# zyang1580/PDA

Measured on AMD Instinct MI355X. Metric: users/sec full-catalogue top-K@50 (eval), higher is better.
Workload: dtype f32; 1 GPU; C3: synthetic 1000000 users x 200000 items, d=128, PDA condition ((elu+1)*pop^0.22) head, masked top-K@50; ranks_seen=1

## Files before the change

### include/pda_hip_experimental.h

```cpp
#ifndef PDA_HIP_EXPERIMENTAL_H
#define PDA_HIP_EXPERIMENTAL_H

#include "pda_hip.h"

#ifdef __cplusplus
extern "C" {
#endif

int pda_score_topk_huge_splits(int n_users_blk, int n_items_local, int d);

int pda_topk_kth_value(const uint64_t* keys, int n_splits, int n_users_blk, int K, int pos, float* out, void* stream);
int pda_topk_remap_items(uint64_t* keys, size_t n_keys, const int32_t* gid, int n_gid, void* stream);
int pda_topk_seed_bounds(const uint64_t* keys, int n_splits, int n_users_blk, int K, int m, float* bounds, void* stream);
int pda_topk_seed_counts(const uint64_t* keys, int n_splits, int n_users_blk, int K, const float* bounds, int n_thr, int32_t* counts,
                         void* stream);
int pda_topk_seed_pick(const float* bounds, const int32_t* counts, int n_thr, int n_users_blk, int K, float* seed, void* stream);
int pda_topk_seed_refine(const uint64_t* keys, int n_splits, int n_users_blk, int K, float* lo, float* hi, float* mid, int32_t* counts,
                         int mode, void* stream);
int pda_score_topk4_phase_f32(const float* U, const float* I_shard, const void* prep, const float* pop_shard, const int32_t* users,
                              int n_users_blk, int item_offset, int n_items_local, int d, const int64_t* hist_indptr,
                              const int32_t* hist_indices, int hist_row_mode, int K, int head, int early_stop, int n_splits,
                              int phase, int warm_tiles, const float* seed, uint64_t* out_keys, void* workspace, void* stream);
int pda_score_topk4_phase_bf16(const uint16_t* U, const uint16_t* I_shard, const void* prep, const float* pop_shard,
                               const int32_t* users, int n_users_blk, int item_offset, int n_items_local, int d,
                               const int64_t* hist_indptr, const int32_t* hist_indices, int hist_row_mode, int K, int head,
                               int early_stop, int n_splits, int phase, int warm_tiles, const float* seed, uint64_t* out_keys,
                               void* workspace, void* stream);

size_t pda_triplet_plan_bytes(int B);
size_t pda_triplet_plan_large_workspace_bytes(int B);
int pda_triplet_plan_large(const int32_t* users, const int32_t* pos, const int32_t* neg, int B, void* plan, void* workspace, void* stream);
size_t pda_bpr_step_plan_scratch_bytes(int B, int d);
int pda_triplet_plan(const int32_t* users, const int32_t* pos, const int32_t* neg, int B, int n_batches, void* plans, void* stream);
int pda_bpr_step_plan_f32(float* U, float* I, const int32_t* users, const int32_t* pos, const int32_t* neg, const float* pos_pop,
                          const float* neg_pop, int B, int d, float regs, float reg_div, float lr, const void* plan, float* scratch,
                          int exact, float* loss_acc, void* stream);
int pda_bpr_step_plan_bf16(uint16_t* U_bf16, uint16_t* I_bf16, float* U_master, float* I_master, const int32_t* users,
                           const int32_t* pos, const int32_t* neg, const float* pos_pop, const float* neg_pop, int B, int d,
                           float regs, float reg_div, float lr, const void* plan, float* scratch, float* loss_acc, void* stream);

int pda_sort_triplets_by_pos(int32_t* users, int32_t* pos, int32_t* neg, float* pos_pop, float* neg_pop, int B,
                             void* stream);
// ... 59 lines not shown
```

### pda_amd/_lib.py

```python
from __future__ import annotations

import ctypes as C
import os

_HERE = os.path.dirname(os.path.abspath(__file__))
LIB_PATH = os.environ.get("PDA_HIP_LIB") or os.path.join(_HERE, "csrc", "libpda_hip.so")

ABI_VERSION = 2
HEAD_RAW, HEAD_POP = 0, 1
HIST_BY_BLOCK_ROW, HIST_BY_USER_ID = 0, 1
UPD_NONE, UPD_SGD_FUSED, UPD_DENSE_GRAD = 0, 1, 2
UPD_ANY_ORDER = 0x100
UPD_USERS_DISTINCT = 0x200
ADAM_REPLAY_FAST = 0x10
MAX_K = 64
TOPK_CAP = 60

_vp, _i, _f, _u64, _sz = C.c_void_p, C.c_int, C.c_float, C.c_uint64, C.c_size_t

class ScorePlan(C.Structure):
    _fields_ = [("path", _i), ("sweep_mode", _i), ("n_splits", _i), ("early_stop", _i), ("order", _i), ("prep_with_pop", _i),
                ("workspace_bytes", _sz), ("keys_rows", _sz)]


# ... 37 lines not shown
    "pda_score_topk4_bf16": (_i, [_vp, _vp, _vp, _vp, _vp, _i, _i, _i, _i, _vp, _vp, _i, _i, _i, _i, _i, _vp, _vp, _vp]),
    "pda_peak_mfma_flops_per_launch": (C.c_double, [_i]),
    "pda_peak_mfma_bf16": (_i, [_vp, _i, _vp]),
    "pda_peak_mfma_bf16_const": (_i, [_vp, _i, _vp]),
    "pda_peak_mfma_lds_flops_per_launch": (C.c_double, [_i]),
    "pda_peak_mfma_lds_bf16": (_i, [_vp, _sz, _vp, _i, _vp]),
    "pda_peak_copy": (_i, [_vp, _vp, _sz, _vp]),
    "pda_topk_kth_value": (_i, [_vp, _i, _i, _i, _i, _vp, _vp]),
    "pda_topk_remap_items": (_i, [_vp, _sz, _vp, _i, _vp]),
    "pda_topk_seed_refine": (_i, [_vp, _i, _i, _i, _vp, _vp, _vp, _vp, _i, _vp]),
    "pda_topk_seed_bounds": (_i, [_vp, _i, _i, _i, _i, _vp, _vp]),
    "pda_topk_seed_counts": (_i, [_vp, _i, _i, _i, _vp, _i, _vp, _vp]),
    "pda_topk_seed_pick": (_i, [_vp, _vp, _i, _i, _i, _vp, _vp]),
    "pda_score_topk4_phase_f32": (_i, [_vp, _vp, _vp, _vp, _vp, _i, _i, _i, _i, _vp, _vp, _i, _i, _i, _i, _i, _i, _i, _vp, _vp, _vp, _vp]),
    "pda_score_topk4_phase_bf16": (_i, [_vp, _vp, _vp, _vp, _vp, _i, _i, _i, _i, _vp, _vp, _i, _i, _i, _i, _i, _i, _i, _vp, _vp, _vp, _vp]),
    "pda_score_topk_plan": (_i, [_i, _i, _i, _i, _i, _i, _i, _i, _vp]),
    "pda_score_topk_huge_splits": (_i, [_i, _i, _i]),
    "pda_score_topk7_workspace_bytes": (_sz, [_i, _i, _i]),
    "pda_score_topk7_f32": (_i, [_vp, _vp, _vp, _vp, _i, _i, _i, _i, _vp, _vp, _i, _i, _i, _vp, _vp, _vp]),
    "pda_score_topk7_bf16": (_i, [_vp, _vp, _vp, _vp, _i, _i, _i, _i, _vp, _vp, _i, _i, _i, _vp, _vp, _vp]),
    "pda_topk_merge": (_i, [_vp, _i, _i, _i, _vp, _vp, _vp, _vp, _vp, _vp, _i, _vp]),
    "pda_bpr_step_f32": (_i, [_vp, _vp, _vp, _vp, _vp, _vp, _vp, _i, _i, _f, _f, _f, _i, _vp, _vp, _vp, _vp, _vp, _vp, _vp]),
    "pda_triplet_plan_bytes": (_sz, [_i]),
    "pda_bpr_step_plan_scratch_bytes": (_sz, [_i, _i]),
    "pda_triplet_plan": (_i, [_vp, _vp, _vp, _i, _i, _vp, _vp]),
    "pda_triplet_plan_large_workspace_bytes": (_sz, [_i]),
    "pda_triplet_plan_large": (_i, [_vp, _vp, _vp, _i, _vp, _vp, _vp]),
    "pda_bpr_step_plan_f32": (_i, [_vp, _vp, _vp, _vp, _vp, _vp, _vp, _i, _i, _f, _f, _f, _vp, _vp, _i, _vp, _vp]),
    "pda_bpr_step_plan_bf16": (_i, [_vp, _vp, _vp, _vp, _vp, _vp, _vp, _vp, _vp, _i, _i, _f, _f, _f, _vp, _vp, _vp, _vp]),
    "pda_sgd_apply_f32": (_i, [_vp, _vp, _vp, _vp, _vp, _vp, _vp, _vp, _i, _i, _f, _vp]),
# ... 101 lines not shown
```

### pda_amd/csrc/pda_score_topk.hip

```cpp
#include "pda_topk_common.h"
#include "pda_hip_temp_pop.h"
#include "pda_hip_pc.h"
#include <cstdlib>

namespace {

using namespace pda_topk;

template <int D, int HEAD, int ABL = 0, bool BF = false>
__global__ void __launch_bounds__(kThreads, (D <= 128 ? 2 : 1)) score_topk_kernel(ScoreArgs a) {
    extern __shared__ __attribute__((aligned(16))) unsigned char smem[];
    float* Bt = reinterpret_cast<float*>(smem);
    uint64_t* lists = reinterpret_cast<uint64_t*>(smem + 32 * D * sizeof(float));

    constexpr int CPR = D / 4;
    constexpr int NLD = (32 * CPR) / kThreads;
    static_assert(NLD >= 1, "embed dim too small for the 256-thread staging pattern");
    constexpr int NC = D / 8;
    static_assert(NC % 2 == 0, "embed dim must be a multiple of 16");

    const int tid = threadIdx.x, lane = tid & 63, wave = tid >> 6;
    const int j = lane & 31, h = lane >> 5;
    const int split = blockIdx.x % a.n_splits, utile = blockIdx.x / a.n_splits;
    const int K = a.K;
// ... 417 lines not shown
                if (a.out_val) a.out_val[(size_t)u * K + lane] = k ? pda_key_val(k) : -INFINITY;
            }
        }
        if (nreal < K && a.out_idx && a.hist_indptr && lane == 0) {
            const int64_t hr = a.hist_row_mode == PDA_HIST_BY_USER_ID ? (int64_t)a.users[u] : (int64_t)u;
            int fill = nreal, prev = -1;
            for (int64_t p = a.hist_indptr[hr]; p < a.hist_indptr[hr + 1] && fill < K; ++p) {
                const int it = a.hist_indices[p];
                if (it != prev) a.out_idx[(size_t)u * K + fill++] = it;
                prev = it;
            }
        }
    }
}

}

int pda_topk::launch_score_bias(const ScoreArgs& a, int d, hipStream_t s) {
    switch (d) {
        case 64: return launch_score<64, PDA_HEAD_BIAS>(a, s);
        case 128: return launch_score<128, PDA_HEAD_BIAS>(a, s);
        case 256: return launch_score<256, PDA_HEAD_BIAS>(a, s);
        default: return PDA_ERR_UNSUPPORTED;
    }
}

int pda_topk::launch_score_pc(const ScoreArgs& a, int d, bool by_g, hipStream_t s) {
    switch (d) {
        case 64: return by_g ? launch_score<64, kHeadPcG>(a, s) : launch_score<64, PDA_HEAD_PC>(a, s);
        case 128: return by_g ? launch_score<128, kHeadPcG>(a, s) : launch_score<128, PDA_HEAD_PC>(a, s);
// ... 63 lines not shown
    if (head != PDA_HEAD_RAW && head != PDA_HEAD_POP) return PDA_ERR_ARG;
    if (head == PDA_HEAD_POP && !pop_shard) return PDA_ERR_ARG;
    if (hist_indptr && !hist_indices) return PDA_ERR_ARG;
    if (n_splits <= 0) n_splits = pda_score_topk_auto_splits(n_users_blk, n_items_local);
    ScoreArgs a{U, I_shard, pop_shard, users, hist_indptr, hist_indices, out_keys,
                n_users_blk, item_offset, n_items_local, hist_row_mode, K, n_splits, nullptr};
    return pda_topk::launch_score_v1(a, d, head, reinterpret_cast<hipStream_t>(stream));
}

extern "C" int pda_topk_merge(const uint64_t* in_keys, int R, int n_users_blk, int K, uint64_t* out_keys,
                              int32_t* out_idx, float* out_val, const int32_t* users, const int64_t* hist_indptr,
                              const int32_t* hist_indices, int hist_row_mode, void* stream) {
    if (!in_keys || R < 1 || n_users_blk <= 0 || K < 1 || K > PDA_MAX_K) return PDA_ERR_ARG;
    if (!out_keys && !out_idx) return PDA_ERR_ARG;
    if (hist_indptr && (!hist_indices || (hist_row_mode == PDA_HIST_BY_USER_ID && !users))) return PDA_ERR_ARG;
    const size_t smem = 4 * (((size_t)R * K + PDA_MAX_K) * sizeof(uint64_t) + (((size_t)R * 4 + 7) & ~(size_t)7));
    if (smem > 160 * 1024) return PDA_ERR_UNSUPPORTED;
    static int attr_set = 0;
    if (!attr_set) {
        if (hipFuncSetAttribute(reinterpret_cast<const void*>(&topk_merge_kernel),
                                hipFuncAttributeMaxDynamicSharedMemorySize, 160 * 1024) != hipSuccess)
            return PDA_ERR_LAUNCH;
        attr_set = 1;
    }
    MergeArgs a{in_keys, out_keys, out_idx, out_val, users, hist_indptr, hist_indices, hist_row_mode, R, n_users_blk, K};
    const int blocks = min((n_users_blk + 3) / 4, 256 * 8);
    hipLaunchKernelGGL(topk_merge_kernel, dim3((unsigned)blocks), dim3(256), smem, reinterpret_cast<hipStream_t>(stream), a);
    PDA_CHECK_LAUNCH();
    return PDA_OK;
}
// ... 1 lines not shown
```

### pda_amd/csrc/pda_score_topk_v4.hip

```cpp
#include "pda_v4_shared.h"
#include <cstdlib>
#include <type_traits>

using namespace pda_topk;

namespace {

constexpr int kCap4 = 57;
constexpr int kRing4 = 128;
constexpr int kWarmTiles = 4;
constexpr int kMainWaves = 8;
#ifndef PDA_W4_ABL
#define PDA_W4_ABL 0
#endif
#ifndef PDA_V4_ABL
#define PDA_V4_ABL 0
#endif
#ifdef PDA_V4_PROF
__device__ unsigned long long pda_prof4[24];
#define PROF_T0(v) const long long v = __builtin_readcyclecounter()
#define PROF_T1(v, slot) prof[slot] += (unsigned long long)(__builtin_readcyclecounter() - v)
#define PROF_INC(slot, x) prof[slot] += (unsigned long long)(x)
#define PROF_FLUSH(first, last) do { if (lane == 0) for (int pq = (first); pq <= (last); ++pq) atomicAdd(&pda_prof4[pq], prof[pq]); } while (0)
#else
// ... 30 lines not shown
    int warm_tiles;
    int warm_sorted;
    uint64_t* handover;
    const unsigned char* rows5;
    const float* meta5;
    const unsigned char* ufrag;
    const float* unorm;
    int prep_hdr_pop;
    int warm_final;
    int warm_shared;
    float* seed_out;
    const int* n_users_dev;
    int lists_empty;
    const float* tailA;
    const float* tailB;
};


template <int D, bool BF>
__global__ void __launch_bounds__(256) prep4_kernel(const void* __restrict__ I, const float* __restrict__ pop, const int* __restrict__ order,
                                                    int n, int n_pad, unsigned char* __restrict__ rows, int* __restrict__ pos_of,
                                                    int* __restrict__ hdr, unsigned char* __restrict__ rows5, int* __restrict__ meta5, u32x4* __restrict__ pinfo,
                                                    int f16img) {
    constexpr int TPR = D / 8, RB = row_bytes(D);
    const int pos = blockIdx.x * (256 / TPR) + threadIdx.x / TPR, e = threadIdx.x % TPR;
    if (pos >= n_pad) return;
    unsigned char* rp = rows + (size_t)pos * RB;
    float ss = 0.f, popv = 1.0f, rs = 0.f;
    int src = -1;
    if (pos < n) {
// ... 336 lines not shown
    for (int q = tid; q < kUserTile * 2 * kWarmTiles; q += kThreads) hmask[q] = 0u;
    __syncthreads();
    if (g.hmask_ws != nullptr) {
        const uint32_t* src = g.hmask_ws + (size_t)blockIdx.x * kUserTile * 2 * kWarmTiles;
        for (int q = tid; q < kUserTile * 2 * kWarmTiles; q += kThreads) hmask[q] = src[q];
    } else if (g.hist_indptr != nullptr && !(PDA_W4_ABL & 1)) {
        warm_hist_walk(g, hmask, utile, split, nwarm, wave, lane);
    }
    f32x4 areg[NC];
#pragma unroll
    for (int c = 0; c < NC; ++c) {
        f32x4 v = {0.f, 0.f, 0.f, 0.f};
        if (row_ok) v = pda_load4<BF>(g.U, (size_t)uid * D + 4 * h + 8 * c);
        areg[c] = v;
    }
    if (g.pred_ws != nullptr) {
        float ss = 0.f;
#pragma unroll
        for (int c = 0; c < NC; ++c) ss += areg[c][0] * areg[c][0] + areg[c][1] * areg[c][1] + areg[c][2] * areg[c][2] + areg[c][3] * areg[c][3];
        ss += __shfl_xor(ss, 32, 64);
        if (h == 0) nul[wave * 32 + j] = sqrtf(ss) * 1.0009765625f * 1.0001f;
    }
    const float* brow = Bt + j * D;
    const int bswz = swz<D>(j);
    uint64_t* my_lists = lists + (size_t)(wave * 32) * CAP;
    constexpr int NHT = 2 * kWarmTiles;
    static_assert(NHT == 8, "eight named half-tile registers below");
    typedef uint32_t u32x16 __attribute__((ext_vector_type(16)));
    u32x16 o0 = 0u, o1 = 0u, o2 = 0u, o3 = 0u, o4 = 0u, o5 = 0u, o6 = 0u, o7 = 0u;
    int i0 = 0, i1 = 0, i2 = 0, i3 = 0, i4 = 0, i5 = 0, i6 = 0, i7 = 0;
// ... 39 lines not shown
#pragma unroll
        for (int r = 0; r < 16; ++r) {
            const int row = (r & 3) + 8 * (r >> 2) + 4 * h;
            float sc = accx[r];
            if constexpr (HEAD == PDA_HEAD_POP) sc = (sc > 0.0f ? sc + 1.0f : __expf(sc)) * pv;
            bool p = okw && (sc >= -INFINITY);
            if (any_hb) {
                const uint32_t hbr = (uint32_t)__shfl((int)hb_mine, row, 64);
                if ((hbr >> j) & 1u) p = false;
            }
            o0[r] = p ? pda_ordf(sc + 0.0f) : 0u;
        }
    }
    const u32x16 ordv[NHT] = {o0, o1, o2, o3, o4, o5, o6, o7};
    const int itemv[NHT] = {i0, i1, i2, i3, i4, i5, i6, i7};
    const int cap_t = (g.warm_sorted || g.handover != nullptr) ? CAP : K;
    auto emit_row = [&](const int r, const uint32_t t, const int c_t) __attribute__((always_inline)) {
        const int row = (r & 3) + 8 * (r >> 2) + 4 * h;
        const int lrow = wave * 32 + row;
        if (j == 0) predt[lrow] = c_t >= K ? pda_unordf(t) : -INFINITY;
        if (__any(c_t > cap_t)) {
#pragma unroll
            for (int k = 0; k < NHT; ++k) {
                const bool p = ordv[k][r] >= t;
                const uint64_t key = ((uint64_t)ordv[k][r] << 32) | (uint64_t)(0xFFFFFFFFu - (uint32_t)itemv[k]);
                append_keys<CAP>(p, lrow, pda_unordf(ordv[k][r]), key, lists, cntl, taul, wave * 32, 32, K, lane);
            }
        } else {
            int run = 0;
#pragma unroll
            for (int k = 0; k < NHT; ++k) {
// ... 85 lines not shown
    }
    pda_wave_sync();
    if (tid == 0) atomicAdd(reinterpret_cast<unsigned long long*>(g.stats + 2), (unsigned long long)(2 * nwarm));
    for (int rr = 0; rr < 32; ++rr) {
        uint64_t* buf = my_lists + rr * CAP;
        if (((PDA_W4_ABL & 4) == 0) && (g.warm_sorted || g.warm_final || (g.handover == nullptr && __builtin_amdgcn_readfirstlane(cntl[wave * 32 + rr]) > K)))
            compact_list<CAP>(buf, &cntl[wave * 32 + rr], &taul[wave * 32 + rr], K, lane);
        const int c = cntl[wave * 32 + rr];
        const int rb = utile * kUserTile + wave * 32 + rr;
        if (g.seed_out != nullptr) {
            uint32_t mn = lane < c ? (uint32_t)(buf[lane] >> 32) : 0xFFFFFFFFu;
#pragma unroll
            for (int o = 32; o >= 1; o >>= 1) mn = min(mn, (uint32_t)__shfl_xor((int)mn, o, 64));
            if (lane == 0 && rb < g.n_users_blk) g.seed_out[rb] = c >= K ? pda_unordf(mn) : -INFINITY;
        }
        if (g.handover != nullptr) {
            if (rb < g.n_users_blk && lane < CAP) g.handover[((size_t)split * g.n_users_blk + rb) * CAP + lane] = lane < c ? buf[lane] : 0ull;
            if (g.warm_final && rb < g.n_users_blk && lane < K) g.out_keys[((size_t)split * g.n_users_blk + rb) * K + lane] = lane < c ? buf[lane] : 0ull;
        } else if (rb < g.n_users_blk && lane < K) {
            const uint64_t k = lane < c ? buf[lane] : 0ull;
            g.out_keys[((size_t)split * g.n_users_blk + rb) * K + lane] = k;
        }
    }
    if (g.pred_ws != nullptr && lane < 32) {
        const int rb = utile * kUserTile + wave * 32 + lane;
        if (rb < g.n_users_blk) {
            g.pred_ws[2 * (size_t)rb] = predt[wave * 32 + lane];
            g.pred_ws[2 * (size_t)rb + 1] = nul[wave * 32 + lane];
        }
    }
}


#include "pda_v4_block_asm.h"
#ifndef PDA_V4_ASM
#define PDA_V4_ASM 1
// ... 1085 lines not shown
    {
        if constexpr (HEAD == PDA_HEAD_POP) {
            if (geometry == 4 && g.sufA == nullptr && g.prep_hdr_pop != 0) return launch_sweep5<D, BF, true, D == 256 ? 128 : 256>(g, stream);
        }
        if constexpr (D <= 128) {
            if (geometry == 3) return launch_sweep4<D, HEAD, BF, 3>(g, stream);
        }
        return launch_sweep4<D, HEAD, BF, 0>(g, stream);
    }
    return PDA_OK;
}

int user_tile4(int d) { return d == 64 ? Geo4<64>::UT : d == 128 ? Geo4<128>::UT : Geo4<256>::UT; }
static bool lists_in_hbm4(int) { return true; }
struct Ws4 {
    size_t lists, bloom, hmask, regroup, handover, ufrag, unorm, seed, total;
};
static Ws4 ws4_layout(int n_users_blk, int d, int n_splits) {
    auto al = [](size_t x) { return (x + 255) & ~(size_t)255; };
    Ws4 w{};
    w.lists = al(pda_score_topk_workspace_bytes(n_users_blk));
    size_t b = w.lists;
    if (lists_in_hbm4(d)) {
        const size_t ut = 1024;
        b += ((size_t)n_users_blk + ut - 1) / ut * (size_t)n_splits * ut * kCap4 * 8 + 256;
    }
    w.bloom = al(b);
    w.hmask = al(w.bloom + (size_t)n_users_blk * 128);
    w.regroup = al(w.hmask + ((size_t)n_users_blk + kUserTile - 1) / kUserTile * (size_t)n_splits * kUserTile * 2 * kWarmTiles * 4);
    w.handover = al(w.regroup + (1024 + 4 * (size_t)n_users_blk) * 4);
    w.total = w.handover + (size_t)n_splits * (size_t)n_users_blk * kCap4 * 8;
    w.ufrag = al(w.total);
    w.unorm = w.ufrag;
    {
        const size_t n_pad = ((size_t)n_users_blk + kUT5 - 1) / kUT5 * kUT5;
        w.unorm = w.ufrag + al(n_pad * 2 * (size_t)d);
        w.total = w.unorm + al(n_pad * 4);
    }
    w.seed = w.total;
    w.total = w.seed + al((size_t)n_users_blk * 4);
    return w;
}
extern "C" size_t pda_score_topk4_workspace_bytes(int n_users_blk, int n_items_local, int d, int n_splits) {
    if (n_users_blk <= 0 || n_items_local <= 0 || (d != 64 && d != 128 && d != 256)) return 0;
    if (n_splits <= 0) n_splits = pda_score_topk4_auto_splits(n_users_blk, n_items_local, d);
    return ws4_layout(n_users_blk, d, n_splits).total;
}

int run_score4(const void* U, const void* I_shard, bool bf16, const void* prep, const float* pop_shard, const int32_t* users,
               int n_users_blk, int item_offset, int n_items_local, int d, const int64_t* hist_indptr, const int32_t* hist_indices,
               int hist_row_mode, int K, int head, int early_stop, int n_splits, uint64_t* out_keys, void* workspace, hipStream_t s,
               int phase = 3, const float* seed = nullptr, int warm_tiles = 0, const int* n_users_dev = nullptr) {
    if (!U || !I_shard || !prep || !users || !out_keys || !workspace) return PDA_ERR_ARG;
    if (n_users_blk <= 0 || n_items_local <= 0 || item_offset < 0) return PDA_ERR_ARG;
    if (K < 1 || K > PDA_MAX_K) return PDA_ERR_ARG;
// ... 33 lines not shown
            early_stop ? sA : nullptr, early_stop ? sB : nullptr, reinterpret_cast<const int*>(pb + L.pos_of),
            reinterpret_cast<unsigned*>(workspace), reinterpret_cast<uint64_t*>(wsb + W.lists), nullptr, nullptr, nullptr, nullptr, nullptr, reinterpret_cast<const int*>(pb + L.hdr), seed, n_users_blk, item_offset, n_items_local, hist_row_mode, K, n_splits, L.n_tiles, warm_tiles,
#ifdef PDA_V4_WARM_SORTED
            1, nullptr, pb + L.rows5, reinterpret_cast<const float*>(pb + L.meta5), nullptr, nullptr, 0};
#else
            (phase == 1 || (L.n_tiles + n_splits - 1) / n_splits <= warm_tiles) ? 1 : 0, nullptr,
            pb + L.rows5, reinterpret_cast<const float*>(pb + L.meta5), nullptr, nullptr, 0};
#endif
    if (phase == 3 && !g.warm_sorted && PDA_V4_HANDOVER_WS) g.handover = reinterpret_cast<uint64_t*>(wsb + W.handover);
    g.ufrag = wsb + W.ufrag;
    g.unorm = reinterpret_cast<const float*>(wsb + W.unorm);
    g.prep_hdr_pop = (head == PDA_HEAD_POP && pop_shard != nullptr) ? 1 : 0;
    g.warm_final = (geometry >= 4 && phase == 3 && g.handover != nullptr && g.prep_hdr_pop && !early_stop) ? 1 : 0;
    g.lists_empty = from_empty ? 1 : 0;
    g.n_users_dev = n_users_dev;
    if (g.prep_hdr_pop) {
        g.tailA = reinterpret_cast<const float*>(pb + L.sufA);
        g.tailB = reinterpret_cast<const float*>(pb + L.sufB);
    }
    if (phase == 3 && n_splits > 1 && seed == nullptr && !warm_per_split && L.n_tiles > n_splits * warm_tiles) {
        g.warm_shared = 1;
        g.seed_out = reinterpret_cast<float*>(wsb + W.seed);
    }
    if (hist_indptr && (phase & 2)) {
        uint32_t* bloom = reinterpret_cast<uint32_t*>(wsb + W.bloom);
        hipLaunchKernelGGL(hist_bloom4_kernel, dim3((unsigned)((n_users_blk + 31) / 32)), dim3(256), 0, s, users, hist_indptr, hist_indices,
                           hist_row_mode, n_users_blk, bloom, reinterpret_cast<const int*>(pb + L.hdr), head == PDA_HEAD_POP ? 1 : 0);
        PDA_CHECK_LAUNCH();
        g.bloom = bloom;
    }
// ... 249 lines not shown

extern "C" int pda_score_topk4_f32(const float* U, const float* I_shard, const void* prep, const float* pop_shard, const int32_t* users,
                                   int n_users_blk, int item_offset, int n_items_local, int d, const int64_t* hist_indptr,
                                   const int32_t* hist_indices, int hist_row_mode, int K, int head, int early_stop, int n_splits,
                                   uint64_t* out_keys, void* workspace, void* stream) {
    return run_score4(U, I_shard, false, prep, pop_shard, users, n_users_blk, item_offset, n_items_local, d, hist_indptr, hist_indices,
                      hist_row_mode, K, head, early_stop, n_splits, out_keys, workspace, reinterpret_cast<hipStream_t>(stream));
}
extern "C" int pda_score_topk4_bf16(const uint16_t* U, const uint16_t* I_shard, const void* prep, const float* pop_shard, const int32_t* users,
                                    int n_users_blk, int item_offset, int n_items_local, int d, const int64_t* hist_indptr,
                                    const int32_t* hist_indices, int hist_row_mode, int K, int head, int early_stop, int n_splits,
                                    uint64_t* out_keys, void* workspace, void* stream) {
    return run_score4(U, I_shard, true, prep, pop_shard, users, n_users_blk, item_offset, n_items_local, d, hist_indptr, hist_indices,
                      hist_row_mode, K, head, early_stop, n_splits, out_keys, workspace, reinterpret_cast<hipStream_t>(stream));
}
```

### pda_amd/csrc/pda_v5_sweep.h

```cpp
#pragma once
#ifdef PDA_V6_LOOP_HEADER
#include PDA_V6_LOOP_HEADER
#else
#include "pda_v6_loop_asm.h"
#endif
#include "pda_v6_free_asm.h"

#ifdef PDA_V5_LOG
__device__ unsigned pda_v5_log[1 << 18];
#define V5LOG(kind, a, b) do { if (lane == 0) { const unsigned i_ = atomicAdd(&pda_v5_log[0], 1u); if (i_ < (1u << 16) - 1u) { \
    pda_v5_log[4 * i_ + 4] = ((unsigned)blockIdx.x << 8) | (unsigned)wave; pda_v5_log[4 * i_ + 5] = (kind); pda_v5_log[4 * i_ + 6] = (a); pda_v5_log[4 * i_ + 7] = (b); } } } while (0)
#else
#define V5LOG(kind, a, b) do {} while (0)
#endif
constexpr int kRing5 = 192;



template <int D, bool BF, bool S16, int UPW>
__global__ void __launch_bounds__(256, 1) sweep5_kernel(Args4 g) {
    [[maybe_unused]] constexpr int HB = half_bytes5(D);
    static_assert(slot_bytes5(D) == Loop6<D, 8>::kSlotBytes, "one LDS image for all loops");
    static_assert(S16, "the loop on v_mfma_f32_32x32x16_bf16 (round 4's first form: 9.16 against 8.07 ms, profiles/README.md) left with round 5; the parameter keeps the kernel's name");
    static_assert((D <= 128 && UPW == 256) || (D == 256 && UPW == 128), "users per wave: 256, or (d = 256) 128 -- 8 blocks x 8 k-steps = 256 AGPRs, one 512-user workgroup per CU");
// ... 17 lines not shown
    const int K = g.K;
    const int nt = split_tiles(g.n_tiles, split, g.n_splits);
    const int wt = warm_tiles_of(g, split);
    const bool starts_empty = g.lists_empty || (g.warm_shared && split > 0);
    const bool warm_final = g.warm_final && !starts_empty;
    const int n_it = max(0, nt - wt);
    const unsigned hend = 2u * (unsigned)n_it;
    if (tid < 72) sync[tid] = (tid < 8 || tid >= 40 || warm_final || starts_empty) ? 0u : 0xFFFFFFFFu;
    if (tid == 0 && blockIdx.x == 0) g.stats[4] = (4u << 28) | (4u << 8) | (1u << 13) | ((BF ? 1u : 0u) << 14) | (unsigned)(D >> 6);
    if (starts_empty) {
        for (int rr = tid; rr < UT; rr += 256) {
            cntl[rr] = 0;
            taul[rr] = utile * UT + rr < g.n_users_blk ? -INFINITY : INFINITY;
        }
        __builtin_amdgcn_fence(__ATOMIC_RELEASE, "workgroup");
    } else if (warm_final) {
        for (int rr = tid; rr < UT; rr += 256) {
            const int rb = utile * UT + rr;
            int c = 0;
            float tau = INFINITY;
            if (rb < g.n_users_blk) {
                const uint64_t kl = lists[(size_t)rr * CAPL + (K - 1)];
                c = K;
                tau = pda_unordf((uint32_t)(kl >> 32));
                if (kl == 0ull) {
                    tau = -INFINITY;
                    for (c = 0; c < K - 1 && lists[(size_t)rr * CAPL + c] != 0ull; ++c) {}
                }
            }
            cntl[rr] = c;
// ... 45 lines not shown
            const int rb = utile * UT + row0 + UBW * u + j;
            eu = fmaxf(eu, rb < g.n_users_blk ? g.unorm[rb] : 0.f);
            seedv[u] = (g.seed != nullptr && rb < g.n_users_blk) ? g.seed[rb] : -INFINITY;
        }
#pragma unroll
        for (int o = 32; o >= 1; o >>= 1) eu = fmaxf(eu, __shfl_xor(eu, o, 64));
        const float numax = eu;
        eu = __int_as_float(__builtin_amdgcn_readfirstlane(__float_as_int(eu * (kEps5 * 1.001f))));
        const unsigned ring_lds = (unsigned)(size_t)(__attribute__((address_space(3))) unsigned char*)tiles;
        const unsigned flags_lds = (unsigned)(size_t)(__attribute__((address_space(3))) unsigned char*)reinterpret_cast<unsigned char*>(sync);
        uint64_t* my_ring = crings + wave * kRing5;
        unsigned ring_n = 0;
        const unsigned t0 = (unsigned)(split + wt * g.n_splits);
        const size_t img = (size_t)g.rows5, meta = (size_t)g.meta5;
        const bool hist_on = g.hist_indptr != nullptr;

        auto thr_of = [&](int u) __attribute__((always_inline)) -> float {
            const float tq = fmaxf(taul[row0 + UBW * u + j], seedv[u]);
            float tf = (tq == INFINITY || tq == -INFINITY) ? tq : tq - fabsf(tq) * 1.52587890625e-5f - 1e-30f;
            return fminf(fmaxf(tf, -1.0e30f), 1.0e30f);
        };
        auto rescore_ring = [&]() __attribute__((always_inline)) {
            const int q = lane % LPC, ci = lane / LPC;
            for (unsigned base = 0; base < ring_n; base += CPP) {
                const bool have = base + (unsigned)ci < ring_n;
                const uint64_t e = have ? my_ring[base + ci] : 0ull;
                const int row = (int)(e >> 32);
                const unsigned pos = (unsigned)e;
                bool valid = have && pos < (unsigned)g.n_items_local;
                const unsigned char* tail = g.rows + (size_t)(valid ? pos : 0u) * RB4 + 2 * D + 32;
// ... 77 lines not shown
                const float o0 = LPC == 8 ? o_other : __int_as_float(__builtin_amdgcn_mov_dpp(__float_as_int(o), 0xB1, 0xF, 0xF, true));
                float sc = o0 + o;
                sc = (sc > 0.0f ? sc + 1.0f : __expf(sc)) * pv;
                const float tt = (valid && q == LPC - 1) ? sc : -INFINITY;
                const int item = g.item_offset + loc;
                bool p = valid && q == LPC - 1 && (tt >= fmaxf(c_tau, c_sd));
                if (hist_on && p) {
                    long long lo = hb, hi2 = he;
                    while (lo < hi2) {
                        const long long mid = (lo + hi2) >> 1;
                        if (g.hist_indices[mid] < item) lo = mid + 1; else hi2 = mid;
                    }
                    if (lo < he && g.hist_indices[lo] == item) p = false;
                }
                const uint64_t key = pda_pack_key(tt, (uint32_t)item);
                if (p) atomicOr(&touched[(row0 + row) >> 5], 1u << ((row0 + row) & 31));
                append_keys<CAPL, true>(p, row0 + row, tt, key, lists, cntl, taul, row0, UPW, K, lane, s_uns);
            }
            n_cand += ring_n;
            ring_n = 0;
        };
        auto extract = [&](unsigned ft) __attribute__((always_inline)) {
            const unsigned T = t0 + (ft >> 1) * (unsigned)g.n_splits;
            const unsigned pos0 = T * 64u + (ft & 1u) * 32u;
            const float2 mt = *reinterpret_cast<const float2*>(g.meta5 + 4 * (size_t)(2u * T + (ft & 1u)));
            const float ct = __builtin_fmaf(eu, mt.y, mt.x);
            const unsigned char* tb = tiles + (ft & (kNSlot5 - 1)) * SS + j * (2 * D);
            auto item_of = [&](int r) __attribute__((always_inline)) -> unsigned {
                return 16u * (r >> 2) + 4u * hh + (r & 3);
            };
            constexpr int NR = 8;
// ... 187 lines not shown
}

template <int D, bool BF, bool S16, int UPW>
int launch_sweep5(const Args4& g, hipStream_t stream) {
    constexpr int UT = 4 * UPW;
    constexpr size_t lds = (size_t)kNSlot5 * slot_bytes5(D) + (size_t)UT * 8 + 4 * kRing5 * 8 + 80 * 4 + 64;
    static_assert(UPW == 256 || D == 256 || 2 * lds <= 160 * 1024, "two workgroups per CU");
    static_assert(lds <= 160 * 1024, "LDS per workgroup");
    static int attr_set = 0;
    if (!attr_set) {
        if (hipFuncSetAttribute(reinterpret_cast<const void*>(&sweep5_kernel<D, BF, S16, UPW>), hipFuncAttributeMaxDynamicSharedMemorySize, (int)lds) != hipSuccess)
            return PDA_ERR_LAUNCH;
        attr_set = 1;
    }
    const int utiles = (g.n_users_blk + UT - 1) / UT, n_pad = utiles * UT;
    hipLaunchKernelGGL((uprep5_kernel<D, BF, S16, UPW>), dim3((unsigned)(((size_t)n_pad * (D / 8) + 255) / 256)), dim3(256), 0, stream, g.U, g.users, g.n_users_blk, n_pad,
                       const_cast<unsigned char*>(g.ufrag), const_cast<float*>(g.unorm));
    PDA_CHECK_LAUNCH();
    hipLaunchKernelGGL((sweep5_kernel<D, BF, S16, UPW>), dim3((unsigned)(utiles * g.n_splits)), dim3(256), lds, stream, g);
    PDA_CHECK_LAUNCH();
    return PDA_OK;
}
```

### pda_amd/ops.py

```python
from __future__ import annotations

import math
import os
from typing import Optional, Tuple

import ctypes as C

import torch

from . import _lib
from ._lib import (HEAD_POP, HEAD_RAW, HIST_BY_BLOCK_ROW, HIST_BY_USER_ID, UPD_ANY_ORDER, UPD_DENSE_GRAD, UPD_NONE, UPD_USERS_DISTINCT,
                   UPD_SGD_FUSED, check, ptr, stream_ptr)

ADAM_BETA1, ADAM_BETA2, ADAM_EPS = 0.9, 0.999, 1e-8


def _need(t: Optional[torch.Tensor], dtype, name: str, optional=False):
    if t is None:
        if optional:
            return None
        raise ValueError(f"{name} is required")
    if not t.is_cuda:
        raise ValueError(f"{name} must live in HBM (cuda tensor); pda_amd has no CPU path")
    if t.dtype != dtype:
# ... 504 lines not shown
        check(fn(ptr(U), ptr(I_shard), ptr(prep), ptr(pop_shard), ptr(users), nu, item_offset, nloc, d,
                 ptr(hist.indptr) if hist else None, ptr(hist.indices) if hist else None, hist.mode if hist else 0,
                 K, head, es, n_splits, ptr(out), ptr(ws), stream_ptr()), "pda_score_topk4")
        if os.environ.get("PDA_CHECK_SWEEP_ERRORS"):
            err = int(ws[0:4].view(torch.int32)[0])
            if err != 0:
                raise RuntimeError("pda_score_topk4: the sweep reported protocol error %d" % err)
        if stats is not None:
            stats["tiles_scored"] = ws[8:16].view(torch.int64)
            stats["pairs_rescored"] = ws[4:8].view(torch.int32)
            stats["tiles_dense"] = ((nloc + 31) // 32) * ((nu + 127) // 128)
            stats["kernel_id"] = ws[16:20].view(torch.int32)
            stats["huge_entries"] = ws[20:24].view(torch.int32)
            stats["huge_free_halftiles"] = ws[28:32].view(torch.int32)
            stats["error"] = ws[0:4].view(torch.int32)
        return out
    if impl == "v2" and prune:
        prep, order = item_prep_ordered(I_shard, pop_shard if head == HEAD_POP else None)
        hist_ord = hist_reordered(hist, prep, order, item_offset, nloc, d) if hist else None
        ws = torch.empty(lib.pda_score_topk_workspace_bytes(nu), dtype=torch.uint8, device=U.device)
        fn = lib.pda_score_topk_ordered_bf16 if bf else lib.pda_score_topk_ordered_f32
        check(fn(ptr(U), ptr(I_shard), ptr(prep), ptr(pop_shard), ptr(users), nu, item_offset,
                                             nloc, d, ptr(hist.indptr) if hist else None,
                                             ptr(hist.indices) if hist else None, ptr(hist_ord), hist.mode if hist else 0,
                                             K, head, 0 if prune == "order" else 1, n_splits, ptr(out), ptr(ws), stream_ptr()),
              "pda_score_topk_ordered")
        if stats is not None:
            stats["tiles_scored"] = ws[8:16].view(torch.int64)
            stats["pairs_rescored"] = ws[4:8].view(torch.int32)
            stats["tiles_dense"] = ((nloc + 31) // 32) * ((nu + 127) // 128)
# ... 72 lines not shown
        stats["error"] = ws[0:4].view(torch.int32)
        stats["fallback_rows"] = ws[24:28].view(torch.int32)
        stats["workspace"] = ws
    return out


GEOMETRY_NAMES = {0: "lds", 3: "many", 4: "huge", 7: "funnel"}


def kernel_identity(word) -> dict:
    w = int(word) & 0xFFFFFFFF
    if w == 0:
        return {"generation": 0}
    return {"generation": w >> 28, "geometry": GEOMETRY_NAMES.get((w >> 8) & 15, "?") if (w >> 28) == 4 else None,
            ("early_stop" if (w >> 28) == 4 else "visiting_order"): bool((w >> 12) & 1), "head": (w >> 13) & 1, "bf16": bool((w >> 14) & 1), "d": (w & 15) * 64}


def topk_merge(keys: torch.Tensor, users=None, hist: Optional[HistoryCSR] = None, want="idx_val"):
    lib = _lib.load()
    keys = _need(keys, torch.int64, "keys")
    R, nu, K = keys.shape
    dev = keys.device
    out_keys = out_idx = out_val = None
    if want == "keys":
        out_keys = torch.empty((nu, K), dtype=torch.int64, device=dev)
    else:
        out_idx = torch.empty((nu, K), dtype=torch.int32, device=dev)
        out_val = torch.empty((nu, K), dtype=torch.float32, device=dev)
    if users is not None:
        users = _need(users, torch.int32, "users")
# ... 847 lines not shown
```

Baseline: 32.05 million users/s.

## Fuse user-image prep into warm phase, drop handover copy, add R=1 unpack

The warm-phase kernel now writes the bf16 user fragment image and user norms itself, so the sweep no longer launches a separate uprep kernel. The final warm phase stores only the per-split K-th value plus the K keys instead of a full CAP-wide handover list. The sweep then reloads a row's list lazily, only the first time that row gains a candidate. A vectorised single-split unpack kernel replaces the shared-memory merge when R==1. Together these aim to cut extra launches and HBM traffic, in exchange for more complex sweep logic (ballot-driven lazy reloads with extra syncs) and new correctness risk in list reconstruction.

Result: faster. 32.42 million users/s, median of 6 (+1.2%).

```diff
diff --git a/include/pda_hip_experimental.h b/include/pda_hip_experimental.h
--- a/include/pda_hip_experimental.h
+++ b/include/pda_hip_experimental.h
@@ -26,6 +26,9 @@
                                const int64_t* hist_indptr, const int32_t* hist_indices, int hist_row_mode, int K, int head,
                                int early_stop, int n_splits, int phase, int warm_tiles, const float* seed, uint64_t* out_keys,
                                void* workspace, void* stream);
+int pda_score_topk4_phase_image_offsets(int n_users_blk, int n_items_local, int d, int n_splits, size_t* offs);
+int pda_score_topk4_phase_user_image(const void* U, int bf16, const int32_t* users, int n_users_blk, int d, void* ufrag, float* unorm,
+                                     void* stream);
 
 size_t pda_triplet_plan_bytes(int B);
 size_t pda_triplet_plan_large_workspace_bytes(int B);
diff --git a/pda_amd/_lib.py b/pda_amd/_lib.py
--- a/pda_amd/_lib.py
+++ b/pda_amd/_lib.py
@@ -75,6 +75,8 @@
     "pda_topk_seed_pick": (_i, [_vp, _vp, _i, _i, _i, _vp, _vp]),
     "pda_score_topk4_phase_f32": (_i, [_vp, _vp, _vp, _vp, _vp, _i, _i, _i, _i, _vp, _vp, _i, _i, _i, _i, _i, _i, _i, _vp, _vp, _vp, _vp]),
     "pda_score_topk4_phase_bf16": (_i, [_vp, _vp, _vp, _vp, _vp, _i, _i, _i, _i, _vp, _vp, _i, _i, _i, _i, _i, _i, _i, _vp, _vp, _vp, _vp]),
+    "pda_score_topk4_phase_image_offsets": (_i, [_i, _i, _i, _i, _vp]),
+    "pda_score_topk4_phase_user_image": (_i, [_vp, _i, _vp, _i, _i, _vp, _vp, _vp]),
     "pda_score_topk_plan": (_i, [_i, _i, _i, _i, _i, _i, _i, _i, _vp]),
     "pda_score_topk_huge_splits": (_i, [_i, _i, _i]),
     "pda_score_topk7_workspace_bytes": (_sz, [_i, _i, _i]),
diff --git a/pda_amd/csrc/pda_score_topk.hip b/pda_amd/csrc/pda_score_topk.hip
--- a/pda_amd/csrc/pda_score_topk.hip
+++ b/pda_amd/csrc/pda_score_topk.hip
@@ -455,6 +455,74 @@
     }
 }
 
+constexpr int kUnpackKeys = 4;
+
+__device__ __forceinline__ void unpack1_fill_row(const MergeArgs& a, size_t u) {
+    const int K = a.K;
+    const uint64_t* row = a.in_keys + u * K;
+    int nreal = 0;
+    for (int p = 0; p < K; ++p) nreal += row[p] != 0ull ? 1 : 0;
+    int32_t* orow = a.out_idx + u * K;
+    for (int p = 0; p < K; ++p)
+        if (row[p] == 0ull) orow[p] = -1;
+    const int64_t hr = a.hist_row_mode == PDA_HIST_BY_USER_ID ? (int64_t)a.users[u] : (int64_t)u;
+    int fill = nreal, prev = -1;
+    for (int64_t p = a.hist_indptr[hr]; p < a.hist_indptr[hr + 1] && fill < K; ++p) {
+        const int it = a.hist_indices[p];
+        if (it != prev) orow[fill++] = it;
+        prev = it;
+    }
+}
+
+__global__ void __launch_bounds__(256) topk_unpack1_kernel(MergeArgs a, size_t total) {
+    typedef uint64_t u64x2 __attribute__((ext_vector_type(2)));
+    typedef int32_t i32x4 __attribute__((ext_vector_type(4)));
+    const size_t g = (size_t)blockIdx.x * 256 + threadIdx.x;
+    const size_t i0 = g * kUnpackKeys;
+    if (i0 >= total) return;
+    const bool fill_on = a.out_idx != nullptr && a.hist_indptr != nullptr;
+    if (i0 + kUnpackKeys <= total) {
+        const u64x2 k01 = *reinterpret_cast<const u64x2*>(a.in_keys + i0), k23 = *reinterpret_cast<const u64x2*>(a.in_keys + i0 + 2);
+        const uint64_t k[kUnpackKeys] = {k01[0], k01[1], k23[0], k23[1]};
+        if (a.out_keys) {
+            *reinterpret_cast<u64x2*>(a.out_keys + i0) = k01;
+            *reinterpret_cast<u64x2*>(a.out_keys + i0 + 2) = k23;
+        }
+        if (a.out_idx == nullptr) return;
+        i32x4 id;
+        f32x4 v;
+#pragma unroll
+        for (int q = 0; q < kUnpackKeys; ++q) {
+            id[q] = k[q] ? pda_key_item(k[q]) : -1;
+            v[q] = k[q] ? pda_key_val(k[q]) : -INFINITY;
+        }
+        if (a.out_val) *reinterpret_cast<f32x4*>(a.out_val + i0) = v;
+        const bool empty = k[0] == 0ull || k[1] == 0ull || k[2] == 0ull || k[3] == 0ull;
+        if (!(fill_on && empty)) {
+            *reinterpret_cast<i32x4*>(a.out_idx + i0) = id;
+            return;
+        }
+        const size_t u0 = i0 / (size_t)a.K;
+        int p = (int)(i0 - u0 * (size_t)a.K);
+        size_t u = u0;
+#pragma unroll
+        for (int q = 0; q < kUnpackKeys; ++q) {
+            if (k[q] != 0ull) a.out_idx[i0 + q] = id[q];
+            else if (p == a.K - 1) unpack1_fill_row(a, u);
+            if (++p == a.K) { p = 0; ++u; }
+        }
+        return;
+    }
+    for (size_t i = i0; i < total; ++i) {
+        const uint64_t k = a.in_keys[i];
+        if (a.out_keys) a.out_keys[i] = k;
+        if (a.out_idx == nullptr) continue;
+        if (a.out_val) a.out_val[i] = k ? pda_key_val(k) : -INFINITY;
+        if (k != 0ull || !fill_on) a.out_idx[i] = k ? pda_key_item(k) : -1;
+        else if ((i + 1) % (size_t)a.K == 0) unpack1_fill_row(a, i / (size_t)a.K);
+    }
+}
+
 }
 
 int pda_topk::launch_score_bias(const ScoreArgs& a, int d, hipStream_t s) {
@@ -548,6 +616,16 @@
     if (!in_keys || R < 1 || n_users_blk <= 0 || K < 1 || K > PDA_MAX_K) return PDA_ERR_ARG;
     if (!out_keys && !out_idx) return PDA_ERR_ARG;
     if (hist_indptr && (!hist_indices || (hist_row_mode == PDA_HIST_BY_USER_ID && !users))) return PDA_ERR_ARG;
+#ifndef PDA_MERGE_R1_GENERAL
+    if (R == 1 && ((reinterpret_cast<uintptr_t>(in_keys) | reinterpret_cast<uintptr_t>(out_keys) | reinterpret_cast<uintptr_t>(out_idx) |
+                    reinterpret_cast<uintptr_t>(out_val)) & 15u) == 0) {
+        MergeArgs a{in_keys, out_keys, out_idx, out_val, users, hist_indptr, hist_indices, hist_row_mode, 1, n_users_blk, K};
+        const size_t total = (size_t)n_users_blk * K, threads = (total + kUnpackKeys - 1) / kUnpackKeys;
+        hipLaunchKernelGGL(topk_unpack1_kernel, dim3((unsigned)((threads + 255) / 256)), dim3(256), 0, reinterpret_cast<hipStream_t>(stream), a, total);
+        PDA_CHECK_LAUNCH();
+        return PDA_OK;
+    }
+#endif
     const size_t smem = 4 * (((size_t)R * K + PDA_MAX_K) * sizeof(uint64_t) + (((size_t)R * 4 + 7) & ~(size_t)7));
     if (smem > 160 * 1024) return PDA_ERR_UNSUPPORTED;
     static int attr_set = 0;
diff --git a/pda_amd/csrc/pda_score_topk_v4.hip b/pda_amd/csrc/pda_score_topk_v4.hip
--- a/pda_amd/csrc/pda_score_topk_v4.hip
+++ b/pda_amd/csrc/pda_score_topk_v4.hip
@@ -68,6 +68,9 @@
     int lists_empty;
     const float* tailA;
     const float* tailB;
+    unsigned char* ufrag_out;
+    float* unorm_out;
+    float* kth_ws;
 };
 
 
@@ -434,6 +437,41 @@
         if (row_ok) v = pda_load4<BF>(g.U, (size_t)uid * D + 4 * h + 8 * c);
         areg[c] = v;
     }
+    if constexpr (HEAD == PDA_HEAD_POP) {
+        if (g.ufrag_out != nullptr && split == 0) {
+            constexpr int NK5 = D / 32;
+            unsigned char* fb = g.ufrag_out + ((size_t)(row_blk >> 4) * (NK5 * 64) + (size_t)(row_blk & 15)) * 16 + 8 * h;
+            float ssc[NC];
+#pragma unroll
+            for (int c = 0; c < NC; ++c) {
+                const f32x4 v = areg[c];
+                uint2 w;
+                w.x = bf16_rne(v[0]) | (bf16_rne(v[1]) << 16);
+                w.y = bf16_rne(v[2]) | (bf16_rne(v[3]) << 16);
+                *reinterpret_cast<uint2*>(fb + ((c >> 2) * 64 + 16 * (c & 3)) * 16) = w;
+                float ss = 0.f;
+#pragma unroll
+                for (int k = 0; k < 4; ++k) {
+                    const float sq = v[k] * v[k];
+                    ss += sq + __shfl_xor(sq, 32, 64);
+                }
+                ssc[c] = ss;
+            }
+#pragma unroll
+            for (int o = NC / 2; o > 0; o >>= 1)
+#pragma unroll
+                for (int c = 0; c < o; ++c) ssc[c] += ssc[c + o];
+            if (h == 0) g.unorm_out[row_blk] = sqrtf(ssc[0]) * 1.0009765625f * 1.0001f;
+            const int utiles_w = (g.n_users_blk + kUserTile - 1) / kUserTile;
+            if (utile == utiles_w - 1) {
+                constexpr int UT5 = D == 256 ? 512 : kUT5;
+                const size_t r0 = (size_t)utiles_w * kUserTile, r1 = ((size_t)g.n_users_blk + UT5 - 1) / UT5 * UT5;
+                const u32x4 z = {0u, 0u, 0u, 0u};
+                for (size_t q = r0 * (2 * D) + (size_t)tid * 16; q < r1 * (2 * D); q += (size_t)kThreads * 16) *reinterpret_cast<u32x4*>(g.ufrag_out + q) = z;
+                for (size_t r = r0 + tid; r < r1; r += kThreads) g.unorm_out[r] = 0.f;
+            }
+        }
+    }
     if (g.pred_ws != nullptr) {
         float ss = 0.f;
 #pragma unroll
@@ -503,7 +541,7 @@
     }
     const u32x16 ordv[NHT] = {o0, o1, o2, o3, o4, o5, o6, o7};
     const int itemv[NHT] = {i0, i1, i2, i3, i4, i5, i6, i7};
-    const int cap_t = (g.warm_sorted || g.handover != nullptr) ? CAP : K;
+    const int cap_t = (g.warm_sorted || g.handover != nullptr || g.warm_final) ? CAP : K;
     auto emit_row = [&](const int r, const uint32_t t, const int c_t) __attribute__((always_inline)) {
         const int row = (r & 3) + 8 * (r >> 2) + 4 * h;
         const int lrow = wave * 32 + row;
@@ -619,12 +657,30 @@
             for (int o = 32; o >= 1; o >>= 1) mn = min(mn, (uint32_t)__shfl_xor((int)mn, o, 64));
             if (lane == 0 && rb < g.n_users_blk) g.seed_out[rb] = c >= K ? pda_unordf(mn) : -INFINITY;
         }
+        if (g.kth_ws != nullptr) continue;
         if (g.handover != nullptr) {
             if (rb < g.n_users_blk && lane < CAP) g.handover[((size_t)split * g.n_users_blk + rb) * CAP + lane] = lane < c ? buf[lane] : 0ull;
             if (g.warm_final && rb < g.n_users_blk && lane < K) g.out_keys[((size_t)split * g.n_users_blk + rb) * K + lane] = lane < c ? buf[lane] : 0ull;
         } else if (rb < g.n_users_blk && lane < K) {
             const uint64_t k = lane < c ? buf[lane] : 0ull;
             g.out_keys[((size_t)split * g.n_users_blk + rb) * K + lane] = k;
+        }
+    }
+    if (g.kth_ws != nullptr) {
+        pda_wave_sync();
+        const int rb0 = utile * kUserTile + wave * 32, nv = max(0, min(32, g.n_users_blk - rb0));
+        if (lane < nv) {
+            const uint64_t kl = my_lists[(size_t)lane * CAP + (K - 1)];
+            g.kth_ws[(size_t)split * g.n_users_blk + rb0 + lane] = cntl[wave * 32 + lane] >= K ? pda_unordf((uint32_t)(kl >> 32)) : -INFINITY;
+        }
+        uint64_t* ob = g.out_keys + ((size_t)split * g.n_users_blk + rb0) * K;
+        const int q64 = 64 / K, r64 = 64 % K;
+        int rr = lane / K, p = lane % K;
+        for (int i = lane; i < nv * K; i += 64) {
+            ob[i] = p < cntl[wave * 32 + rr] ? my_lists[(size_t)rr * CAP + p] : 0ull;
+            rr += q64;
+            p += r64;
+            if (p >= K) { p -= K; ++rr; }
         }
     }
     if (g.pred_ws != nullptr && lane < 32) {
@@ -1740,7 +1796,7 @@
 int user_tile4(int d) { return d == 64 ? Geo4<64>::UT : d == 128 ? Geo4<128>::UT : Geo4<256>::UT; }
 static bool lists_in_hbm4(int) { return true; }
 struct Ws4 {
-    size_t lists, bloom, hmask, regroup, handover, ufrag, unorm, seed, total;
+    size_t lists, bloom, hmask, regroup, handover, ufrag, unorm, seed, kth, total;
 };
 static Ws4 ws4_layout(int n_users_blk, int d, int n_splits) {
     auto al = [](size_t x) { return (x + 255) & ~(size_t)255; };
@@ -1765,6 +1821,8 @@
     }
     w.seed = w.total;
     w.total = w.seed + al((size_t)n_users_blk * 4);
+    w.kth = w.total;
+    w.total = w.kth + al((size_t)n_splits * (size_t)n_users_blk * 4);
     return w;
 }
 extern "C" size_t pda_score_topk4_workspace_bytes(int n_users_blk, int n_items_local, int d, int n_splits) {
@@ -1828,6 +1886,18 @@
     g.warm_final = (geometry >= 4 && phase == 3 && g.handover != nullptr && g.prep_hdr_pop && !early_stop) ? 1 : 0;
     g.lists_empty = from_empty ? 1 : 0;
     g.n_users_dev = n_users_dev;
+#ifndef PDA_V5_HANDOVER
+    if (g.warm_final && geometry == 4) {
+        g.handover = nullptr;
+        g.kth_ws = reinterpret_cast<float*>(wsb + W.kth);
+    }
+#endif
+#ifndef PDA_V5_UPREP
+    if (geometry == 4 && phase == 3 && g.prep_hdr_pop && !early_stop && n_users_dev == nullptr && (L.n_tiles + n_splits - 1) / n_splits > warm_tiles) {
+        g.ufrag_out = wsb + W.ufrag;
+        g.unorm_out = reinterpret_cast<float*>(wsb + W.unorm);
+    }
+#endif
     if (g.prep_hdr_pop) {
         g.tailA = reinterpret_cast<const float*>(pb + L.sufA);
         g.tailB = reinterpret_cast<const float*>(pb + L.sufB);
@@ -2107,3 +2177,31 @@
     return run_score4(U, I_shard, true, prep, pop_shard, users, n_users_blk, item_offset, n_items_local, d, hist_indptr, hist_indices,
                       hist_row_mode, K, head, early_stop, n_splits, out_keys, workspace, reinterpret_cast<hipStream_t>(stream));
 }
+
+extern "C" int pda_score_topk4_phase_image_offsets(int n_users_blk, int n_items_local, int d, int n_splits, size_t* offs) {
+    if (n_users_blk <= 0 || n_items_local <= 0 || (d != 64 && d != 128 && d != 256) || !offs) return PDA_ERR_ARG;
+    if (n_splits <= 0) n_splits = pda_score_topk4_auto_splits(n_users_blk, n_items_local, d);
+    const Ws4 W = ws4_layout(n_users_blk, d, n_splits);
+    const size_t ut = d == 256 ? 512 : kUT5;
+    offs[0] = W.ufrag;
+    offs[1] = W.unorm;
+    offs[2] = W.kth;
+    offs[3] = ((size_t)n_users_blk + ut - 1) / ut * ut;
+    return PDA_OK;
+}
+extern "C" int pda_score_topk4_phase_user_image(const void* U, int bf16, const int32_t* users, int n_users_blk, int d, void* ufrag, float* unorm,
+                                                void* stream) {
+    if (!U || !users || !ufrag || !unorm || n_users_blk <= 0) return PDA_ERR_ARG;
+    if (d != 64 && d != 128 && d != 256) return PDA_ERR_UNSUPPORTED;
+    hipStream_t s = reinterpret_cast<hipStream_t>(stream);
+    const size_t ut = d == 256 ? 512 : kUT5, n_pad = ((size_t)n_users_blk + ut - 1) / ut * ut;
+#define PDA_UIMG_(DD, BFV, UPWV)                                                                                                                \
+    hipLaunchKernelGGL((uprep5_kernel<DD, BFV, true, UPWV>), dim3((unsigned)((n_pad * (DD / 8) + 255) / 256)), dim3(256), 0, s, U, users, n_users_blk, \
+                       (int)n_pad, reinterpret_cast<unsigned char*>(ufrag), unorm)
+    if (d == 64) { if (bf16) PDA_UIMG_(64, true, 256); else PDA_UIMG_(64, false, 256); }
+    else if (d == 128) { if (bf16) PDA_UIMG_(128, true, 256); else PDA_UIMG_(128, false, 256); }
+    else { if (bf16) PDA_UIMG_(256, true, 128); else PDA_UIMG_(256, false, 128); }
+#undef PDA_UIMG_
+    PDA_CHECK_LAUNCH();
+    return PDA_OK;
+}
diff --git a/pda_amd/csrc/pda_v5_sweep.h b/pda_amd/csrc/pda_v5_sweep.h
--- a/pda_amd/csrc/pda_v5_sweep.h
+++ b/pda_amd/csrc/pda_v5_sweep.h
@@ -55,6 +55,23 @@
             taul[rr] = utile * UT + rr < g.n_users_blk ? -INFINITY : INFINITY;
         }
         __builtin_amdgcn_fence(__ATOMIC_RELEASE, "workgroup");
+    } else if (warm_final && g.kth_ws != nullptr) {
+        for (int rr = tid; rr < UT; rr += 256) {
+            const int rb = utile * UT + rr;
+            int c = 0;
+            float tau = INFINITY;
+            if (rb < g.n_users_blk) {
+                tau = g.kth_ws[(size_t)split * g.n_users_blk + rb];
+                c = K;
+                if (tau == -INFINITY) {
+                    const uint64_t* row = g.out_keys + ((size_t)split * g.n_users_blk + rb) * K;
+                    for (c = 0; c < K && row[c] != 0ull; ++c) {}
+                }
+            }
+            cntl[rr] = c;
+            taul[rr] = tau;
+        }
+        __builtin_amdgcn_fence(__ATOMIC_RELEASE, "workgroup");
     } else if (warm_final) {
         for (int rr = tid; rr < UT; rr += 256) {
             const int rb = utile * UT + rr;
@@ -130,6 +147,7 @@
         const unsigned t0 = (unsigned)(split + wt * g.n_splits);
         const size_t img = (size_t)g.rows5, meta = (size_t)g.meta5;
         const bool hist_on = g.hist_indptr != nullptr;
+        const bool lazy_rows = warm_final && g.kth_ws != nullptr;
 
         auto thr_of = [&](int u) __attribute__((always_inline)) -> float {
             const float tq = fmaxf(taul[row0 + UBW * u + j], seedv[u]);
@@ -237,7 +255,20 @@
                     if (lo < he && g.hist_indices[lo] == item) p = false;
                 }
                 const uint64_t key = pda_pack_key(tt, (uint32_t)item);
-                if (p) atomicOr(&touched[(row0 + row) >> 5], 1u << ((row0 + row) & 31));
+                bool first = false;
+                if (p) first = (atomicOr(&touched[(row0 + row) >> 5], 1u << ((row0 + row) & 31)) & (1u << ((row0 + row) & 31))) == 0u;
+                if (lazy_rows) {
+                    uint64_t need = __ballot(first);
+                    if (need != 0ull) {
+                        while (need != 0ull) {
+                            const int lr = row0 + __builtin_amdgcn_readlane(row, __builtin_ctzll(need));
+                            need &= need - 1ull;
+                            const int c_r = cntl[lr];
+                            if (lane < c_r) lists[(size_t)lr * CAPL + lane] = g.out_keys[((size_t)split * g.n_users_blk + (size_t)(utile * UT + lr)) * K + lane];
+                        }
+                        list_sync<true>();
+                    }
+                }
                 append_keys<CAPL, true>(p, row0 + row, tt, key, lists, cntl, taul, row0, UPW, K, lane, s_uns);
             }
             n_cand += ring_n;
@@ -455,9 +486,11 @@
         attr_set = 1;
     }
     const int utiles = (g.n_users_blk + UT - 1) / UT, n_pad = utiles * UT;
-    hipLaunchKernelGGL((uprep5_kernel<D, BF, S16, UPW>), dim3((unsigned)(((size_t)n_pad * (D / 8) + 255) / 256)), dim3(256), 0, stream, g.U, g.users, g.n_users_blk, n_pad,
-                       const_cast<unsigned char*>(g.ufrag), const_cast<float*>(g.unorm));
-    PDA_CHECK_LAUNCH();
+    if (g.ufrag_out == nullptr) {
+        hipLaunchKernelGGL((uprep5_kernel<D, BF, S16, UPW>), dim3((unsigned)(((size_t)n_pad * (D / 8) + 255) / 256)), dim3(256), 0, stream, g.U, g.users, g.n_users_blk, n_pad,
+                           const_cast<unsigned char*>(g.ufrag), const_cast<float*>(g.unorm));
+        PDA_CHECK_LAUNCH();
+    }
     hipLaunchKernelGGL((sweep5_kernel<D, BF, S16, UPW>), dim3((unsigned)(utiles * g.n_splits)), dim3(256), lds, stream, g);
     PDA_CHECK_LAUNCH();
     return PDA_OK;
diff --git a/pda_amd/ops.py b/pda_amd/ops.py
--- a/pda_amd/ops.py
+++ b/pda_amd/ops.py
@@ -542,6 +542,8 @@
             stats["huge_entries"] = ws[20:24].view(torch.int32)
             stats["huge_free_halftiles"] = ws[28:32].view(torch.int32)
             stats["error"] = ws[0:4].view(torch.int32)
+            stats["workspace"] = ws
+            stats["n_splits"] = n_splits
         return out
     if impl == "v2" and prune:
         prep, order = item_prep_ordered(I_shard, pop_shard if head == HEAD_POP else None)
@@ -644,6 +646,27 @@
         return {"generation": 0}
     return {"generation": w >> 28, "geometry": GEOMETRY_NAMES.get((w >> 8) & 15, "?") if (w >> 28) == 4 else None,
             ("early_stop" if (w >> 28) == 4 else "visiting_order"): bool((w >> 12) & 1), "head": (w >> 13) & 1, "bf16": bool((w >> 14) & 1), "d": (w & 15) * 64}
+
+
+def huge_image_offsets(nu: int, nloc: int, d: int, n_splits: int):
+    offs = (C.c_size_t * 4)()
+    check(_lib.load().pda_score_topk4_phase_image_offsets(nu, nloc, d, n_splits, C.cast(offs, C.c_void_p)), "pda_score_topk4_phase_image_offsets")
+    return int(offs[0]), int(offs[1]), int(offs[2]), int(offs[3])
+
+
+def huge_user_image(U: torch.Tensor, users: torch.Tensor):
+    lib = _lib.load()
+    bf = U.dtype == torch.bfloat16
+    U = _need(U, torch.bfloat16 if bf else torch.float32, "U")
+    users = _need(users, torch.int32, "users")
+    d, nu = U.shape[1], users.numel()
+    ut = 512 if d == 256 else 1024
+    n_pad = -(-nu // ut) * ut
+    ufrag = torch.empty(n_pad * 2 * d, dtype=torch.uint8, device=U.device)
+    unorm = torch.empty(n_pad, dtype=torch.float32, device=U.device)
+    check(lib.pda_score_topk4_phase_user_image(ptr(U), 1 if bf else 0, ptr(users), nu, d, ptr(ufrag), ptr(unorm), stream_ptr()),
+          "pda_score_topk4_phase_user_image")
+    return ufrag, unorm
 
 
 def topk_merge(keys: torch.Tensor, users=None, hist: Optional[HistoryCSR] = None, want="idx_val"):
```
